# SandAI-org/MagiAttention

Measured on AMD Instinct MI355X. Metric: attention TFLOPS/sec fwd+bwd (whole-job; per-GPU = value/n_gpus); cp scaling at seqlen 64k, higher is better.
Workload: dtype bf16; 1 GPU; dense_causal_64k_h32_d128; seqlen=65536, heads=32, kv_heads=32, head_dim=128, mask=causal, global_batch=1, parallelism=cp1

## Files before the change

### magi_attention/csrc/ffa_bwd.hip

```cpp

#include <hip/hip_runtime.h>
#include <math.h>
#include <stdlib.h>

#include "../../include/magi_ffa.h"
#include "ffa_device.h"

#define BWD_BN 32
#define BWD_BM 32

DEV_INLINE bool wave_alive(int m0, int qe) { return m0 < qe; }

DEV_INLINE void glds16_untracked(const void* gsrc, int lds_byte) {
  const int m0v = __builtin_amdgcn_readfirstlane(lds_byte);
  asm volatile("s_mov_b32 m0, %0\n\ts_nop 0\n\tglobal_load_lds_dwordx4 %1, off"
               :: "s"(m0v), "v"(gsrc) : "memory", "m0");
}

struct BwdParams {
  const bf16_t* dout;
  const bf16_t* q;
  const bf16_t* k;
  const bf16_t* v;
  const void* out;
  const float* lse;
  float* dq;
  float* dk;
  float* dv;
  float* dpsum;
  const int* q_ranges;
  const int* k_ranges;
  const int* attn_type_map;
  int hq, hk, gqa;
  float scale;
  float softcap;
  long long total_q, total_k;
  int head_major;
  int work_nx, work_ny, work_nz;
  int head_mult;
  int head_off;
  int n_heads_launch;
  const int* seg_starts;
};

template <bool OUT_F32>
__global__ __launch_bounds__(256) void bwd_preprocess_kernel(BwdParams p, int d,
                                                             long long n_rows) {
  const long long row = (long long)blockIdx.x * 4 + (threadIdx.x >> 6);
  if (row >= n_rows) return;
  const int lane = threadIdx.x & 63;
  const int per = d / 64;
  const bf16_t* do_p = p.dout + row * d;
  float acc = 0.f;
  for (int e = 0; e < per; ++e) {
    const int idx = lane * per + e;
    const float dov = (float)do_p[idx];
    float ov;
    if (OUT_F32)
      ov = ((const float*)p.out)[row * d + idx];
    else
      ov = (float)((const bf16_t*)p.out)[row * d + idx];
    acc += dov * ov;
  }
#pragma unroll
  for (int s = 32; s > 0; s >>= 1) acc += __shfl_xor(acc, s, 64);
  if (lane == 0) p.dpsum[row] = acc;
}


template <int D, bool HAS_SOFTCAP, int MODE, int WAVES>
__global__ __launch_bounds__(64 * WAVES, WAVES == 8 ? 2 : 1)
void ffa_bwd_dkv_kernel(BwdParams p) {
  static_assert(WAVES == 4 || (WAVES == 8 && D != 192), "unsupported shape");
  constexpr int NBUF = (MODE != 0 && WAVES == 8) ? 3 : 2;
  constexpr bool WANT_DV = MODE != 2;
  constexpr bool WANT_DK = MODE != 1;
  constexpr bool V_IN_LDS = MODE == 0;
  constexpr int DF = D / 16;
  constexpr int DT = D / 32;
  constexpr int ROWB = (D == 192) ? 512 : D * 2;
  constexpr int ROWE = ROWB / 2;
  constexpr int VSLOTS = D / 8;
  constexpr int SW32M = ROWB / 32 - 1;
  auto swz = [](int row, int byte_off) {
    return byte_off ^ ((row & SW32M) << 5);
  };
  const long long work_total =
      (long long)p.work_nx * p.work_ny * p.work_nz;
  const long long grid_span = (long long)gridDim.x * gridDim.y * gridDim.z;
  const long long w_first = blockIdx.x +
      (long long)gridDim.x * (blockIdx.y + (long long)gridDim.y * blockIdx.z);
  for (long long w = w_first; w < work_total; w += grid_span) {
  const int wx = (int)(w % p.work_nx);
  const long long w2 = w / p.work_nx;
  const int wy = (int)(w2 % p.work_ny);
  const int wz = (int)(w2 / p.work_ny);
  const int ri = wz;
  const int hidx = p.head_major ? wx : wy;
  const int h = p.head_off + hidx * p.head_mult;
  const int wb = p.head_major ? wy : wx;
  const int ks = p.k_ranges[2 * ri], ke = p.k_ranges[2 * ri + 1];
  const int nblk0 = ks + wb * (BWD_BN * WAVES);
  if (nblk0 >= ke) continue;
  const int seg0 = p.seg_starts ? p.seg_starts[ri] : ri;
  const int seg1 = p.seg_starts ? p.seg_starts[ri + 1] : ri + 1;
  int qs, qe, atype;

  const int tid = threadIdx.x;
  const int lane = tid & 63;
  const int wave = tid >> 6;
  if (WAVES == 8 && wave >= 4) asm volatile("s_setprio 1");

  const int lo32 = lane & 31;
  const int hi = lane >> 5;

  const int n0 = nblk0 + wave * BWD_BN;
  const bool wave_live = n0 < ke;

  const float sl2 = HAS_SOFTCAP ? p.softcap * 1.4426950408889634f
                                : p.scale * 1.4426950408889634f;
  const float cap_pre = HAS_SOFTCAP ? p.scale / p.softcap : 0.f;
  const float log2e = 1.4426950408889634f;

  const int kh = h / p.gqa;
  const size_t k_pitch = (size_t)p.hk * D;
  const size_t q_pitch = (size_t)p.hq * D;

  constexpr int QITER =
      (V_IN_LDS && D == 128 && WAVES == 8) ? BWD_BM : 2 * BWD_BM;
  constexpr int NSUB = QITER / BWD_BM;
  constexpr int KVLDS = V_IN_LDS ? 2 * WAVES * BWD_BN * ROWB : 0;
  constexpr int LSELDS = V_IN_LDS ? 0 : NBUF * 2 * QITER * 4;
  static_assert(NBUF * 2 * QITER * ROWB + LSELDS + KVLDS <= 163840,
                "LDS budget");
  __shared__ __attribute__((aligned(16))) char smem[
      NBUF * 2 * QITER * ROWB + LSELDS + KVLDS];
  auto lds_q = [&](int buf) -> __bf16* {
    return (__bf16*)(smem + (2 * buf) * QITER * ROWB);
  };
  auto lds_do = [&](int buf) -> __bf16* {
    return (__bf16*)(smem + (2 * buf + 1) * QITER * ROWB);
  };
  auto lds_lse = [&](int buf) -> float* {
    return (float*)(smem + NBUF * 2 * QITER * ROWB + buf * 2 * QITER * 4);
  };
  __bf16* lds_kt = (__bf16*)(smem + NBUF * 2 * QITER * ROWB + LSELDS) +
                   wave * BWD_BN * ROWE;
  __bf16* lds_vt = (__bf16*)(smem + NBUF * 2 * QITER * ROWB + LSELDS +
                             KVLDS / 2) +
                   wave * BWD_BN * ROWE;

  const int krow = n0 + lo32;
  const int kcl = min(krow, ke - 1);
  const bf16_t* kp_row = p.k + (size_t)kcl * k_pitch + (size_t)kh * D + hi * 8;
  bf16x8 kfA[V_IN_LDS ? 1 : DF], vfA[(WANT_DK && !V_IN_LDS) ? DF : 1];
  if constexpr (!V_IN_LDS) {
    const bf16_t* vp = p.v + (size_t)kcl * k_pitch + (size_t)kh * D;
#pragma unroll
    for (int dd = 0; dd < DF; ++dd) {
      kfA[dd] = *(const bf16x8*)(kp_row - hi * 8 + dd * 16 + hi * 8);
      if constexpr (WANT_DK)
        vfA[dd] = *(const bf16x8*)(vp + dd * 16 + hi * 8);
    }
  }
  constexpr int ROWS_PER_GLDS_V = 1024 / ROWB;
  if constexpr (V_IN_LDS) {
#pragma unroll
    for (int gi = 0; gi < BWD_BN / ROWS_PER_GLDS_V; ++gi) {
      const int r0v = ROWS_PER_GLDS_V * gi;
      const int r = r0v + lane / (ROWB / 16);
// ... 268 lines not shown
              else
                bnext = tr16_frag(tbase + rb0 + (dcoln ^ sw0),
                                  tbase + rb1 + (dcoln ^ sw1));
            }
            acc[j >> 1] = __builtin_amdgcn_mfma_f32_32x32x16_bf16(
                (j & 1) ? a1 : a0, bcur, acc[j >> 1], 0, 0, 0);
            bcur = bnext;
          }
        };
        if constexpr (MODE == 1) {
          pipe_mm(do_base, cframe_to_afrag(pv, 0), cframe_to_afrag(pv, 1),
                  acc_dv);
        } else if constexpr (MODE == 2) {
          pipe_mm(q_base, cframe_to_afrag(dsv, 0), cframe_to_afrag(dsv, 1),
                  acc_dk);
        } else {
          bf16x8 pa0 = cframe_to_afrag(pv, 0);
          bf16x8 pa1 = cframe_to_afrag(pv, 1);
          bf16x8 da0 = cframe_to_afrag(dsv, 0);
          bf16x8 da1 = cframe_to_afrag(dsv, 1);
#pragma unroll
          for (int dt = 0; dt < DT; ++dt) {
            const int dcol = (dt * 32 + 16 * qhalf) * 2;
            bf16x8 bdo = tr16_frag(do_base + rb0 + (dcol ^ sw0),
                                   do_base + rb1 + (dcol ^ sw1));
            acc_dv[dt] = __builtin_amdgcn_mfma_f32_32x32x16_bf16(
                pa0, bdo, acc_dv[dt], 0, 0, 0);
            bf16x8 bq = tr16_frag(q_base + rb0 + (dcol ^ sw0),
                                  q_base + rb1 + (dcol ^ sw1));
            acc_dk[dt] = __builtin_amdgcn_mfma_f32_32x32x16_bf16(
                da0, bq, acc_dk[dt], 0, 0, 0);
            bf16x8 bdo1 = tr16_frag(do_base + rb2 + (dcol ^ sw2),
                                    do_base + rb3 + (dcol ^ sw3));
            acc_dv[dt] = __builtin_amdgcn_mfma_f32_32x32x16_bf16(
                pa1, bdo1, acc_dv[dt], 0, 0, 0);
            bf16x8 bq1 = tr16_frag(q_base + rb2 + (dcol ^ sw2),
                                   q_base + rb3 + (dcol ^ sw3));
            acc_dk[dt] = __builtin_amdgcn_mfma_f32_32x32x16_bf16(
                da1, bq1, acc_dk[dt], 0, 0, 0);
          }
        }
      }
    }
    }
    cur = (NBUF == 3) ? (cur == 2 ? 0 : cur + 1) : (cur ^ 1);
  }
  __syncthreads();
  }

  if (wave_live) {
#pragma unroll
  for (int r = 0; r < 16; ++r) {
    const int kr = n0 + crow(r, hi);
    if (kr >= ke) continue;
    float* dkp = p.dk + (size_t)kr * k_pitch + (size_t)kh * D;
    float* dvp = p.dv + (size_t)kr * k_pitch + (size_t)kh * D;
#pragma unroll
    for (int dt = 0; dt < DT; ++dt) {
      if constexpr (WANT_DK) {
        if (acc_dk[dt][r] != 0.f)
          unsafeAtomicAdd(dkp + dt * 32 + lo32, acc_dk[dt][r]);
      }
      if constexpr (WANT_DV) {
        if (acc_dv[dt][r] != 0.f)
          unsafeAtomicAdd(dvp + dt * 32 + lo32, acc_dv[dt][r]);
      }
    }
  }
  }
  if constexpr (MODE == 0) break;
  }
}


template <int D, bool HAS_SOFTCAP, int WAVES>
__global__ __launch_bounds__(64 * WAVES, WAVES == 8 ? 1 : 2)
void ffa_bwd_dq_kernel(BwdParams p) {
  static_assert(WAVES == 4 || (WAVES == 8 && D != 192), "unsupported shape");
  constexpr int NBUF = WAVES == 8 ? 3 : 2;
  constexpr int DF = D / 16;
  constexpr int DT = D / 32;
  constexpr int ROWB = (D == 192) ? 512 : D * 2;
  constexpr int ROWE = ROWB / 2;
  constexpr int VSLOTS = D / 8;
  constexpr int SW32M = ROWB / 32 - 1;
  auto swz = [](int row, int byte_off) {
    return byte_off ^ ((row & SW32M) << 5);
  };
  const long long work_total =
      (long long)p.work_nx * p.work_ny * p.work_nz;
  const long long grid_span = (long long)gridDim.x * gridDim.y * gridDim.z;
  for (long long w = blockIdx.x +
           (long long)gridDim.x * (blockIdx.y + (long long)gridDim.y * blockIdx.z);
       w < work_total; w += grid_span) {
  const int wx = (int)(w % p.work_nx);
  const long long w2 = w / p.work_nx;
  const int wy = (int)(w2 % p.work_ny);
  const int wz = (int)(w2 / p.work_ny);
  const int ri = wz;
  const int h = p.head_major ? wx : wy;
  const int wb_lin = p.head_major ? wy : wx;
  const int qs = p.q_ranges[2 * ri], qe = p.q_ranges[2 * ri + 1];
  const int nqb = (qe - qs + BWD_BM * WAVES - 1) / (BWD_BM * WAVES);
  if (wb_lin >= nqb) continue;
  const int seg0 = p.seg_starts ? p.seg_starts[ri] : ri;
  const int seg1 = p.seg_starts ? p.seg_starts[ri + 1] : ri + 1;
  const int at0 = p.attn_type_map ? p.attn_type_map[seg0] : 0;
  const int wb = (at0 == 1 || at0 == 3) ? nqb - 1 - wb_lin : wb_lin;
  const int mblk0 = qs + wb * (BWD_BM * WAVES);
  int ks, ke, atype;

  const int tid = threadIdx.x;
  const int lane = tid & 63;
  const int wave = tid >> 6;
  if (WAVES == 8 && wave >= 4) asm volatile("s_setprio 1");

  const int lo32 = lane & 31;
  const int hi = lane >> 5;

  const int m0 = mblk0 + wave * BWD_BM;
  const int qrow = m0 + lo32;
  const bool qvalid = qrow < qe && m0 < qe;
  const int qcl = qvalid ? qrow : (qe - 1);

  const float sl2 = HAS_SOFTCAP ? p.softcap * 1.4426950408889634f
                                : p.scale * 1.4426950408889634f;
  const float cap_pre = HAS_SOFTCAP ? p.scale / p.softcap : 0.f;
  const float log2e = 1.4426950408889634f;

  const int kh = h / p.gqa;
  const size_t k_pitch = (size_t)p.hk * D;
  const size_t q_pitch = (size_t)p.hq * D;

  constexpr int KITER = 2 * BWD_BN;
  static_assert(NBUF * 2 * KITER * ROWB <= 163840, "LDS budget");
  __shared__ __attribute__((aligned(16))) char smem[NBUF * 2 * KITER * ROWB];
  auto lds_k = [&](int buf) -> __bf16* {
    return (__bf16*)(smem + (2 * buf) * KITER * ROWB);
  };
  auto lds_v = [&](int buf) -> __bf16* {
    return (__bf16*)(smem + (2 * buf + 1) * KITER * ROWB);
  };

  bf16x8 qf[DF], dof[DF];
  {
    const bf16_t* qp = p.q + (size_t)qcl * q_pitch + (size_t)h * D;
    const bf16_t* dp = p.dout + (size_t)qcl * q_pitch + (size_t)h * D;
#pragma unroll
    for (int dd = 0; dd < DF; ++dd) {
      qf[dd] = *(const bf16x8*)(qp + dd * 16 + hi * 8);
      dof[dd] = *(const bf16x8*)(dp + dd * 16 + hi * 8);
    }
  }
  const float lse_q = qvalid ? p.lse[(size_t)qrow * p.hq + h] : INFINITY;
  const float dpsum_q = qvalid ? p.dpsum[(size_t)qrow * p.hq + h] : 0.f;
  const bool row_live = qvalid && lse_q != INFINITY && lse_q != -INFINITY;

  const int mlast = min(mblk0 + BWD_BM * WAVES, qe) - 1;
  int k_lo = 0, k_hi = 0, wk_lo = 0, wk_hi = 0;
  auto seg_bounds = [&]() {
    k_lo = ks; k_hi = ke;
    if (atype == 1 || atype == 3) k_hi = min(k_hi, mlast + (ke - qe) + 1);
    if (atype == 2 || atype == 3) k_lo = max(k_lo, mblk0 + (ks - qs));
    wk_lo = ks; wk_hi = ke;
    if (atype == 1 || atype == 3)
      wk_hi = min(wk_hi, min(m0 + BWD_BM, qe) - 1 + (ke - qe) + 1);
    if (atype == 2 || atype == 3) wk_lo = max(wk_lo, m0 + (ks - qs));
  };

  f32x16 acc_dq[DT];
#pragma unroll
  for (int dt = 0; dt < DT; ++dt) acc_dq[dt] = (f32x16)(0.f);

  constexpr int ROWS_PER_GLDS = 1024 / ROWB;
  static_assert(KITER / WAVES >= ROWS_PER_GLDS, "stage rows per wave");
  constexpr int GLDS_PER_WAVE = (KITER / WAVES) / ROWS_PER_GLDS;
  auto stage_glds = [&](int buf, int n0x) {
#pragma unroll
    for (int gi = 0; gi < GLDS_PER_WAVE; ++gi) {
      const int r0 = (KITER / WAVES) * wave + ROWS_PER_GLDS * gi;
      const int r = r0 + lane / (ROWB / 16);
      const int c = lane % (ROWB / 16);
      const int kr = min(n0x + r, ke - 1);
      int cs = c ^ ((r & SW32M) << 1);
      if (cs >= VSLOTS) cs = 0;
      const int csw = cs * 8;
      __builtin_amdgcn_global_load_lds(
          (const __attribute__((address_space(1))) unsigned int*)(
              p.k + (size_t)kr * k_pitch + (size_t)kh * D + csw),
          (__attribute__((address_space(3))) unsigned int*)&lds_k(buf)[r0 * ROWE],
          16, 0, 0);
      __builtin_amdgcn_global_load_lds(
          (const __attribute__((address_space(1))) unsigned int*)(
              p.v + (size_t)kr * k_pitch + (size_t)kh * D + csw),
          (__attribute__((address_space(3))) unsigned int*)&lds_v(buf)[r0 * ROWE],
          16, 0, 0);
    }
  };

  constexpr int GOPS = 2 * GLDS_PER_WAVE;
  int cur = 0;
  for (int seg = seg0; seg < seg1; ++seg) {
  ks = p.k_ranges[2 * seg];
  ke = p.k_ranges[2 * seg + 1];
  atype = p.attn_type_map ? p.attn_type_map[seg] : 0;
  if (ke <= ks) continue;
  seg_bounds();
  if (k_lo >= k_hi) continue;
  cur = 0;
  stage_glds(0, k_lo);
  if constexpr (NBUF == 3) stage_glds(1, k_lo + KITER);

  for (int n0 = k_lo; n0 < k_hi; n0 += KITER) {
    pipe_barrier<NBUF == 3 ? GOPS : 0>();
    if constexpr (NBUF == 3) {
      stage_glds(cur == 0 ? 2 : cur - 1, n0 + 2 * KITER);
    } else {
      if (n0 + KITER < k_hi) stage_glds(cur ^ 1, n0 + KITER);
    }
#pragma unroll
    for (int sub = 0; sub < 2; ++sub) {
    const int ns = n0 + sub * BWD_BN;
    if (ns >= k_hi) break;
    const __bf16* lkb = lds_k(cur) + sub * BWD_BN * ROWE;
    const __bf16* lvb = lds_v(cur) + sub * BWD_BN * ROWE;

    if (wave_alive(m0, qe) && ns + BWD_BN > wk_lo && ns < wk_hi) {
      f32x16 sA = (f32x16)(0.f), dpA = (f32x16)(0.f);
#pragma unroll
      for (int dd = 0; dd < DF; ++dd) {
        const int off = swz(lo32, lo32 * ROWB + dd * 32 + hi * 16);
        bf16x8 kf = *(const bf16x8*)((const char*)lkb + off);
        bf16x8 vf = *(const bf16x8*)((const char*)lvb + off);
        sA = __builtin_amdgcn_mfma_f32_32x32x16_bf16(kf, qf[dd], sA, 0, 0, 0);
        dpA = __builtin_amdgcn_mfma_f32_32x32x16_bf16(vf, dof[dd], dpA, 0, 0, 0);
      }

      float dsv[16];
      const bool interior =
          (qrow < qe) && row_live && (ns >= ks) && (ns + BWD_BN <= ke) &&
          !((atype == 1 || atype == 3) && (ns + BWD_BN - 1 > m0 + (ke - qe))) &&
          !((atype == 2 || atype == 3) && (ns < m0 + 31 + (ks - qs)));
      if (__all(interior) && !HAS_SOFTCAP) {
        const float lsc = lse_q * log2e;
#pragma unroll
        for (int r = 0; r < 16; ++r) {
          const float pij = fast_exp2(sA[r] * sl2 - lsc);
          dsv[r] = pij * (dpA[r] - dpsum_q) * p.scale;
        }
      } else {
#pragma unroll
        for (int r = 0; r < 16; ++r) {
          const int kk = ns + crow(r, hi);
          bool ok = row_live && kk < ke && kk >= ks;
          if (atype == 1 || atype == 3) ok = ok && (kk - qrow <= ke - qe);
          if (atype == 2 || atype == 3) ok = ok && (kk - qrow >= ks - qs);
          float sv = sA[r];
          float dscale = p.scale;
          float t;
          if (HAS_SOFTCAP) {
            const float th = tanhf(sv * cap_pre);
            t = th * sl2;
            dscale = p.scale * (1.f - th * th);
          } else {
            t = sv * sl2;
          }
          const float pij = ok ? fast_exp2(t - lse_q * log2e) : 0.f;
          dsv[r] = pij * (dpA[r] - dpsum_q) * dscale;
        }
      }

      bf16x8 dsa0 = cframe_to_afrag(dsv, 0);
      bf16x8 dsa1 = cframe_to_afrag(dsv, 1);
      {
        const int qhalf2 = (lane >> 4) & 1;
        const int jrow = (lane & 15) >> 2;
        const int row0 = 8 * hi + jrow;
        const int row1 = 8 * hi + 4 + jrow;
        const int k_base = (int)(unsigned long long)(
            (__attribute__((address_space(3))) const char*)lkb);
        const int lane8 = (lane & 3) * 8;
        const int sw0 = (row0 & SW32M) << 5;
        const int sw1 = (row1 & SW32M) << 5;
        const int rb0 = row0 * ROWB + lane8;
        const int rb1 = row1 * ROWB + lane8;
        const int sw2 = ((row0 + 16) & SW32M) << 5;
        const int sw3 = ((row1 + 16) & SW32M) << 5;
        const int rb2 = (row0 + 16) * ROWB + lane8;
        const int rb3 = (row1 + 16) * ROWB + lane8;
        bf16x8 bcur = tr16_frag(k_base + rb0 + ((16 * qhalf2 * 2) ^ sw0),
                                k_base + rb1 + ((16 * qhalf2 * 2) ^ sw1));
#pragma unroll
        for (int j = 0; j < 2 * DT; ++j) {
          bf16x8 bnext = bcur;
          if (j + 1 < 2 * DT) {
            const int dcoln = (((j + 1) >> 1) * 32 + 16 * qhalf2) * 2;
            if ((j + 1) & 1)
              bnext = tr16_frag(k_base + rb2 + (dcoln ^ sw2),
                                k_base + rb3 + (dcoln ^ sw3));
            else
              bnext = tr16_frag(k_base + rb0 + (dcoln ^ sw0),
                                k_base + rb1 + (dcoln ^ sw1));
          }
          acc_dq[j >> 1] = __builtin_amdgcn_mfma_f32_32x32x16_bf16(
              (j & 1) ? dsa1 : dsa0, bcur, acc_dq[j >> 1], 0, 0, 0);
          bcur = bnext;
        }
      }
    }
    }
    cur = (NBUF == 3) ? (cur == 2 ? 0 : cur + 1) : (cur ^ 1);
  }
  __syncthreads();
  }

#pragma unroll
  for (int r = 0; r < 16; ++r) {
    const int qr = m0 + crow(r, hi);
    if (qr >= qe) continue;
    float* dst = p.dq + (size_t)qr * q_pitch + (size_t)h * D;
#pragma unroll
    for (int dt = 0; dt < DT; ++dt) {
      const float val = acc_dq[dt][r];
      if (val != 0.f) unsafeAtomicAdd(dst + dt * 32 + lo32, val);
    }
  }
  }
}


extern "C" int magi_ffa_bwd_preprocess(const magi_ffa_bwd_args* a) {
  if (!a || !a->dout || !a->out || !a->dpsum) return -1;
  BwdParams p{};
  p.dout = (const bf16_t*)a->dout;
  p.out = a->out;
  p.dpsum = a->dpsum;
  const long long n_rows = a->total_q * a->hq;
  if (n_rows == 0) return 0;
  dim3 grid((unsigned)((n_rows + 3) / 4)), block(256);
  hipStream_t s = (hipStream_t)a->stream;
  if (a->out_is_fp32)
    hipLaunchKernelGGL((bwd_preprocess_kernel<true>), grid, block, 0, s, p,
                       a->d, n_rows);
  else
    hipLaunchKernelGGL((bwd_preprocess_kernel<false>), grid, block, 0, s, p,
                       a->d, n_rows);
  return (int)hipGetLastError();
}

static int fill_bwd_params(const magi_ffa_bwd_args* a, BwdParams* p) {
  if (!a || !a->dout || !a->q || !a->k || !a->v || !a->lse) return -1;
  if (a->d != 64 && a->d != 128 && a->d != 192) return -2;
  if (a->hq % a->hk != 0) return -3;
  if (a->n_ranges <= 0) return 1;
  p->dout = (const bf16_t*)a->dout;
  p->q = (const bf16_t*)a->q;
  p->k = (const bf16_t*)a->k;
  p->v = (const bf16_t*)a->v;
  p->out = a->out;
  p->lse = a->lse;
  p->dq = a->dq;
  p->dk = a->dk;
  p->dv = a->dv;
  p->dpsum = a->dpsum;
  p->q_ranges = a->q_ranges;
  p->k_ranges = a->k_ranges;
  p->attn_type_map = a->attn_type_map;
  p->hq = a->hq;
  p->hk = a->hk;
  p->gqa = a->hq / a->hk;
  p->scale = a->softmax_scale;
  p->softcap = a->softcap;
  p->total_q = a->total_q;
  p->total_k = a->total_k;
  p->seg_starts = a->seg_starts;
  p->head_mult = 1;
  p->head_off = 0;
  p->n_heads_launch = a->hq;
  if (a->cu_margin & 0xFFFF0000) {
    p->head_mult = (a->cu_margin >> 24) & 0xFF;
    p->head_off = (a->cu_margin >> 16) & 0xFF;
    p->n_heads_launch = a->hq / p->head_mult;
  }
  return 0;
}

static int env_int(const char* name, int dflt) {
  const char* e = getenv(name);
  return e ? atoi(e) : dflt;
}

static dim3 cap_grid(dim3 grid, int margin, int wg_per_cu) {
  if (margin <= 0) return grid;
  const long long total = (long long)grid.x * grid.y * grid.z;
  long long cap = (long long)(256 - margin) * wg_per_cu;
  if (cap < 1) cap = 1;
  if (cap > total) cap = total;
  return dim3((unsigned)cap, 1, 1);
}

struct BwdKnobs {
  int head_major;
  int bigseq;
};

static BwdKnobs dq_knobs(const magi_ffa_bwd_args* a) {
  const int hm = ((long long)a->total_k * a->d * 4 <= (16 << 20)) ? 1 : 0;
  return {env_int("MAGI_BWD_HEAD_MAJOR", hm),
          env_int("MAGI_BWD_DQ_BIGSEQ", 8192)};
}

template <int D>
static void launch_dq(int waves, bool sc, dim3 grid, hipStream_t s,
                      const BwdParams& p) {
#define GO(SC, W)                                                          \
  hipLaunchKernelGGL((ffa_bwd_dq_kernel<D, SC, W>), grid, dim3(64 * W), 0, \
                     s, p)
  if constexpr (D != 192) {
    if (waves == 8) {
      if (sc) GO(true, 8); else GO(false, 8);
      return;
    }
  }
  if (sc) GO(true, 4); else GO(false, 4);
#undef GO
}

extern "C" int magi_ffa_bwd_dq(const magi_ffa_bwd_args* a) {
  BwdParams p;
  int rc = fill_bwd_params(a, &p);
  if (rc) return rc > 0 ? 0 : rc;
  const BwdKnobs knobs = dq_knobs(a);
  p.head_major = knobs.head_major;
  const int W = (a->d != 192 && a->max_seqlen_k >= knobs.bigseq) ? 8 : 4;
  if (a->n_ranges > 65535) return -5;
  const int qspan = BWD_BM * W;
  const int qblocks = (int)((a->total_q + qspan - 1) / qspan);
  dim3 grid = p.head_major ? dim3(a->hq, qblocks, (unsigned)a->n_ranges)
                           : dim3(qblocks, a->hq, (unsigned)a->n_ranges);
  p.work_nx = grid.x; p.work_ny = grid.y; p.work_nz = grid.z;
  grid = cap_grid(grid, a->cu_margin & 0xFFFF, W == 4 ? 2 : 1);
  hipStream_t s = (hipStream_t)a->stream;
  const bool sc = a->softcap > 0.f;
  if (a->d == 64) launch_dq<64>(W, sc, grid, s, p);
  else if (a->d == 192) launch_dq<192>(W, sc, grid, s, p);
  else launch_dq<128>(W, sc, grid, s, p);
  return (int)hipGetLastError();
}

static BwdKnobs dkv_knobs() {
  return {env_int("MAGI_BWD_HEAD_MAJOR", 1), env_int("MAGI_BWD_BIGSEQ", 1024)};
}

template <int D, int MODE>
static void launch_dkv(int waves, bool sc, dim3 grid, hipStream_t s,
                       const BwdParams& p) {
#define GO(SC, W)                                                        \
  hipLaunchKernelGGL((ffa_bwd_dkv_kernel<D, SC, MODE, W>), grid,         \
                     dim3(64 * W), 0, s, p)
  if constexpr (D != 192) {
    if (waves == 8) {
      if (sc) GO(true, 8); else GO(false, 8);
      return;
    }
  }
// ... 49 lines not shown
```

### magi_attention/csrc/ffa_device.h

```cpp
#pragma once

#include <hip/hip_runtime.h>

using f32x16 = __attribute__((ext_vector_type(16))) float;
using bf16x8 = __attribute__((ext_vector_type(8))) __bf16;
using bf16_t = __bf16;

#define DEV_INLINE __device__ __forceinline__

template <int VM>
DEV_INLINE void pipe_barrier() {
  asm volatile("s_waitcnt vmcnt(%0)\n\ts_waitcnt lgkmcnt(0)\n\ts_barrier"
               :: "n"(VM) : "memory");
}

DEV_INLINE float warp_xor32(float v) { return __shfl_xor(v, 32, 64); }

DEV_INLINE unsigned pack_bf16_pair(float lo, float hi) {
  unsigned r;
  asm("v_cvt_pk_bf16_f32 %0, %1, %2" : "=v"(r) : "v"(lo), "v"(hi));
  return r;
}

DEV_INLINE float fast_exp2(float x) { return __builtin_amdgcn_exp2f(x); }

DEV_INLINE int crow(int r, int hi) { return (r & 3) + 8 * (r >> 2) + 4 * hi; }

DEV_INLINE bf16x8 tr16_frag(int a0, int a1) {
  typedef __attribute__((ext_vector_type(4))) __bf16 bf16x4_;
  bf16x4_ v0 = __builtin_amdgcn_ds_read_tr16_b64_v4bf16(
      (__attribute__((address_space(3))) bf16x4_*)(unsigned)a0);
  bf16x4_ v1 = __builtin_amdgcn_ds_read_tr16_b64_v4bf16(
      (__attribute__((address_space(3))) bf16x4_*)(unsigned)a1);
  union {
    bf16x4_ h[2];
    bf16x8 v;
  } r;
  r.h[0] = v0;
  r.h[1] = v1;
  return r.v;
}

DEV_INLINE bf16x8 cframe_to_afrag(const float* val, int tt) {
  unsigned c0 = pack_bf16_pair(val[8 * tt + 0], val[8 * tt + 1]);
  unsigned c1 = pack_bf16_pair(val[8 * tt + 2], val[8 * tt + 3]);
  unsigned c2 = pack_bf16_pair(val[8 * tt + 4], val[8 * tt + 5]);
  unsigned c3 = pack_bf16_pair(val[8 * tt + 6], val[8 * tt + 7]);
  {
    auto r2 = __builtin_amdgcn_permlane32_swap(c0, c2, false, false);
    c0 = r2[0];
    c2 = r2[1];
  }
  {
    auto r2 = __builtin_amdgcn_permlane32_swap(c1, c3, false, false);
    c1 = r2[0];
    c3 = r2[1];
  }
  union {
    unsigned u[4];
    bf16x8 v;
  } cvt;
  cvt.u[0] = c0;
  cvt.u[1] = c1;
  cvt.u[2] = c2;
  cvt.u[3] = c3;
  return cvt.v;
}


DEV_INLINE unsigned char to_fp8(float x) {
  union {
    short s;
    unsigned char b[2];
  } r;
  r.s = __builtin_amdgcn_cvt_pk_fp8_f32(x, 0.f, 0, false);
  return r.b[0];
}

DEV_INLINE long cframe_to_afrag_fp8(const float* val, int tt) {
  union {
    unsigned char b[4];
    unsigned u;
  } A, B;
#pragma unroll
  for (int j = 0; j < 4; ++j) {
    A.b[j] = to_fp8(val[8 * tt + j]);
    B.b[j] = to_fp8(val[8 * tt + 4 + j]);
  }
  auto r2 = __builtin_amdgcn_permlane32_swap(A.u, B.u, false, false);
  return ((long)(unsigned)r2[1] << 32) | (unsigned)r2[0];
}
```

### magi_attention/csrc/ffa_fwd.hip

```cpp

#include <hip/hip_runtime.h>
#include <math.h>

#include "../../include/magi_ffa.h"
#include "ffa_device.h"

#define FFA_BM 128
#define FFA_BN 32
#define LOCK_GRAN 128

struct FwdParams {
  const bf16_t* q;
  const bf16_t* k;
  const bf16_t* v;
  float* out_f32;
  bf16_t* out_bf16;
  float* lse;
  const int* q_ranges;
  const int* k_ranges;
  const int* attn_type_map;
  int* locks;
  float* max_logits;
  const int* qk_starts;
  int hq, hk, gqa;
  int head_major;
  int work_nx, work_ny, work_nz;
  int n_lock_slots;
  float scale;
  float softcap;
  long long total_q, total_k;
};

template <int D, bool HAS_SOFTCAP, bool ATOMIC, bool OUT_BF16, int WAVES,
          int NBUF = 2>
__global__ __launch_bounds__(64 * WAVES, 8 / WAVES) void ffa_fwd_kernel(FwdParams p) {
  constexpr int DF = D / 16;
  constexpr int DT = D / 32;
  const long long work_total =
      (long long)p.work_nx * p.work_ny * p.work_nz;
  const long long grid_span = (long long)gridDim.x * gridDim.y * gridDim.z;
  for (long long w = blockIdx.x +
           (long long)gridDim.x * (blockIdx.y + (long long)gridDim.y * blockIdx.z);
       w < work_total; w += grid_span) {
  const int wx = (int)(w % p.work_nx);
  const long long w2 = w / p.work_nx;
  const int wy = (int)(w2 % p.work_ny);
  const int wz = (int)(w2 / p.work_ny);
  const int ri = p.head_major ? wz : wy;
  const int h = p.head_major ? wx : wz;
  const int mb = p.head_major ? wy : wx;
  const int qs = p.q_ranges[2 * ri], qe = p.q_ranges[2 * ri + 1];
  const int m0 = qs + mb * (32 * WAVES);
  if (m0 >= qe) continue;
  const int seg0 = p.qk_starts ? p.qk_starts[ri] : ri;
  const int seg1 = p.qk_starts ? p.qk_starts[ri + 1] : ri + 1;
  int ks, ke, atype;

  const int lane = threadIdx.x & 63;
  const int wave = threadIdx.x >> 6;
  if (WAVES == 8 && wave >= 4) asm volatile("s_setprio 1");

  const int lo32 = lane & 31;
  const int hi = lane >> 5;

  const int q0 = m0 + wave * 32;
  const int qrow = q0 + lo32;
  const bool qvalid = (qrow < qe) && (q0 < qe);
  const bool qvalid_any = q0 < qe;
  const int qclamp = qvalid ? qrow : (qe - 1);

  const float sl2 = HAS_SOFTCAP ? p.softcap * 1.4426950408889634f
                                : p.scale * 1.4426950408889634f;
  const float cap_pre = HAS_SOFTCAP ? p.scale / p.softcap : 0.f;

  int n_lo = 0, n_hi = 0, b_lo = 0, b_hi = 0;
  auto seg_bounds = [&]() {
    n_lo = ks; n_hi = ke;
    if (ke > ks && q0 < qe) {
      const int qhiw = min(q0 + 31, qe - 1);
      if (atype == 1 || atype == 3) n_hi = min(n_hi, qhiw + (ke - qe) + 1);
      if (atype == 2 || atype == 3) n_lo = max(n_lo, q0 + (ks - qs));
    } else {
      n_hi = n_lo;
    }
    b_lo = ks; b_hi = ke;
    if (ke > ks && m0 < qe) {
      const int qhib = min(m0 + 32 * WAVES - 1, qe - 1);
      if (atype == 1 || atype == 3) b_hi = min(b_hi, qhib + (ke - qe) + 1);
      if (atype == 2 || atype == 3) b_lo = max(b_lo, m0 + (ks - qs));
    } else {
      b_hi = b_lo;
    }
  };
  constexpr int ROWB = (D == 192) ? 512 : D * 2;
  constexpr int ROWE = ROWB / 2;
  constexpr int VSLOTS = D / 8;
  constexpr int SW32M = ROWB / 32 - 1;
  auto swz = [](int row, int byte_off) {
    return byte_off ^ ((row & SW32M) << 5);
  };
  constexpr int KITER = 2 * FFA_BN;
  __shared__ __attribute__((aligned(16))) char fsmem[NBUF * 2 * KITER * ROWB];
  auto lds_k = [&](int buf) -> __bf16* {
    return (__bf16*)(fsmem + (2 * buf) * KITER * ROWB);
  };
  auto lds_v = [&](int buf) -> __bf16* {
    return (__bf16*)(fsmem + (2 * buf + 1) * KITER * ROWB);
  };

  bf16x8 qf[DF];
  {
    const bf16_t* qp = p.q + (size_t)qclamp * p.hq * D + (size_t)h * D;
#pragma unroll
    for (int dd = 0; dd < DF; ++dd)
      qf[dd] = *(const bf16x8*)(qp + dd * 16 + hi * 8);
  }

  const int kh = h / p.gqa;
  const size_t k_pitch = (size_t)p.hk * D;
  const bf16_t* kbase = p.k + (size_t)kh * D;
  const bf16_t* vbase = p.v + (size_t)kh * D;

  float m_run = -INFINITY;
  float l_run = 0.f;
  f32x16 acc_o[DT];
#pragma unroll
  for (int dt = 0; dt < DT; ++dt) acc_o[dt] = (f32x16)(0.f);

  constexpr int ROWS_PER_GLDS = 1024 / ROWB;
  static_assert(KITER / WAVES >= ROWS_PER_GLDS, "stage rows per wave");
  constexpr int GLDS_PER_WAVE = (KITER / WAVES) / ROWS_PER_GLDS;
  constexpr int GOPS = 2 * GLDS_PER_WAVE;
  auto stage_glds = [&](int buf, int n0x) {
#pragma unroll
    for (int gi = 0; gi < GLDS_PER_WAVE; ++gi) {
      const int r0 = (KITER / WAVES) * wave + ROWS_PER_GLDS * gi;
      const int r = r0 + lane / (ROWB / 16);
      const int c = lane % (ROWB / 16);
      const int kr = min(n0x + r, ke - 1);
      int cs = c ^ ((r & SW32M) << 1);
      if (cs >= VSLOTS) cs = 0;
      const int csw = cs * 8;
      __builtin_amdgcn_global_load_lds(
          (const __attribute__((address_space(1))) unsigned int*)(
              kbase + (size_t)kr * k_pitch + csw),
          (__attribute__((address_space(3))) unsigned int*)&lds_k(buf)[r0 * ROWE],
          16, 0, 0);
      __builtin_amdgcn_global_load_lds(
          (const __attribute__((address_space(1))) unsigned int*)(
              vbase + (size_t)kr * k_pitch + csw),
          (__attribute__((address_space(3))) unsigned int*)&lds_v(buf)[r0 * ROWE],
          16, 0, 0);
    }
  };

  int cur = 0;

  auto sub_body = [&](int ns, const __bf16* lkb, const __bf16* lvb) {
    const bool live = (ns + FFA_BN > n_lo) && (ns < n_hi) && qvalid_any;
    if (!live) return;

    f32x16 s = (f32x16)(0.f);
    {
#pragma unroll
      for (int dd = 0; dd < DF; ++dd) {
        bf16x8 kf = *(const bf16x8*)(
            (const char*)lkb + swz(lo32, lo32 * ROWB + dd * 32 + hi * 16));
        s = __builtin_amdgcn_mfma_f32_32x32x16_bf16(kf, qf[dd], s, 0, 0, 0);
      }
    }

    const bool interior =
        (q0 + 31 < qe) && (ns >= n_lo) && (ns + FFA_BN <= n_hi) &&
        !((atype == 1 || atype == 3) && (ns + FFA_BN - 1 > q0 + (ke - qe))) &&
        !((atype == 2 || atype == 3) && (ns < q0 + 31 + (ks - qs)));
    float t[16];
    float mx = -INFINITY;
    if (interior) {
#pragma unroll
      for (int r = 0; r < 16; ++r) {
        float sv = s[r];
        if (HAS_SOFTCAP) sv = tanhf(sv * cap_pre);
        t[r] = sv * sl2;
        mx = fmaxf(mx, t[r]);
      }
    } else {
#pragma unroll
      for (int r = 0; r < 16; ++r) {
        const int kk = ns + crow(r, hi);
        bool ok = qvalid && (kk >= n_lo) && (kk < n_hi);
        if (atype == 1 || atype == 3) ok = ok && (kk - qrow <= ke - qe);
        if (atype == 2 || atype == 3) ok = ok && (kk - qrow >= ks - qs);
        float sv = s[r];
        if (HAS_SOFTCAP) sv = tanhf(sv * cap_pre);
        t[r] = ok ? sv * sl2 : -INFINITY;
        mx = fmaxf(mx, t[r]);
      }
    }
    mx = fmaxf(mx, warp_xor32(mx));

    const float m_new = fmaxf(m_run, mx);
    const float defer_thr = p.max_logits ? 0.f : 8.f;
    const bool need_rescale =
        (m_new > m_run + defer_thr) ||
        (m_run == -INFINITY && m_new != -INFINITY);
    float m_use;
    float alpha;
    if (!__any(need_rescale)) {
      m_use = (m_run == -INFINITY) ? 0.f : m_run;
      alpha = 1.f;
    } else {
      m_use = (m_new == -INFINITY) ? 0.f : m_new;
      alpha = (m_run == -INFINITY) ? 0.f : fast_exp2(m_run - m_use);
      m_run = m_new;
    }

    float pr[16];
    float psum = 0.f;
#pragma unroll
    for (int r = 0; r < 16; ++r) {
      pr[r] = fast_exp2(t[r] - m_use);
      psum += pr[r];
    }
    l_run = l_run * alpha + (psum + warp_xor32(psum));

    if (__any(alpha != 1.f)) {
#pragma unroll
      for (int r = 0; r < 16; ++r) {
        const int src = crow(r, hi);
        const float aq = __uint_as_float(
            __builtin_amdgcn_ds_bpermute(src << 2, __float_as_uint(alpha)));
#pragma unroll
        for (int dt = 0; dt < DT; ++dt) acc_o[dt][r] *= aq;
      }
    }

    bf16x8 pa[2];
#pragma unroll
    for (int tt = 0; tt < 2; ++tt) {
      unsigned c0 = pack_bf16_pair(pr[8 * tt + 0], pr[8 * tt + 1]);
      unsigned c1 = pack_bf16_pair(pr[8 * tt + 2], pr[8 * tt + 3]);
      unsigned c2 = pack_bf16_pair(pr[8 * tt + 4], pr[8 * tt + 5]);
      unsigned c3 = pack_bf16_pair(pr[8 * tt + 6], pr[8 * tt + 7]);
      {
        auto r2 = __builtin_amdgcn_permlane32_swap(c0, c2, false, false);
        c0 = r2[0];
        c2 = r2[1];
      }
      {
        auto r2 = __builtin_amdgcn_permlane32_swap(c1, c3, false, false);
        c1 = r2[0];
        c3 = r2[1];
      }
      union {
        unsigned u[4];
        bf16x8 v;
      } cvt;
      cvt.u[0] = c0;
      cvt.u[1] = c1;
      cvt.u[2] = c2;
      cvt.u[3] = c3;
      pa[tt] = cvt.v;
    }

    {
      const int qhalf = (lane >> 4) & 1;
      const int jrow = (lane & 15) >> 2;
      const int v_base = (int)(unsigned long long)(
          (__attribute__((address_space(3))) const char*)lvb);
      const int lane8 = (lane & 3) * 8;
#pragma unroll
      for (int tt = 0; tt < 2; ++tt) {
        const int row0 = 16 * tt + 8 * hi + jrow;
        const int row1 = row0 + 4;
        const int sw0 = (row0 & SW32M) << 5;
        const int sw1 = (row1 & SW32M) << 5;
        const int rb0 = v_base + row0 * ROWB + lane8;
        const int rb1 = v_base + row1 * ROWB + lane8;
#pragma unroll
        for (int dt = 0; dt < DT; ++dt) {
          const int dcol = (dt * 32 + 16 * qhalf) * 2;
          bf16x8 bv = tr16_frag(rb0 + (dcol ^ sw0), rb1 + (dcol ^ sw1));
          acc_o[dt] =
              __builtin_amdgcn_mfma_f32_32x32x16_bf16(pa[tt], bv, acc_o[dt], 0, 0, 0);
        }
      }
    }
  };

  bool any_seg = false;
  for (int seg = seg0; seg < seg1; ++seg) {
    ks = p.k_ranges[2 * seg];
    ke = p.k_ranges[2 * seg + 1];
    atype = p.attn_type_map ? p.attn_type_map[seg] : 0;
    if (ke <= ks) continue;
    seg_bounds();
    if (b_lo >= b_hi) continue;
    any_seg = true;
    cur = 0;
    stage_glds(0, b_lo);
    if constexpr (NBUF == 3) stage_glds(1, b_lo + KITER);
    for (int n0 = b_lo; n0 < b_hi; n0 += KITER) {
      pipe_barrier<NBUF == 3 ? GOPS : 0>();
      if constexpr (NBUF == 3) {
        stage_glds(cur == 0 ? 2 : cur - 1, n0 + 2 * KITER);
      } else {
        if (n0 + KITER < b_hi) stage_glds(cur ^ 1, n0 + KITER);
      }
#pragma unroll
      for (int sub = 0; sub < 2; ++sub) {
        const int ns = n0 + sub * FFA_BN;
        if (ns >= b_hi) break;
        sub_body(ns, lds_k(cur) + sub * FFA_BN * ROWE,
                 lds_v(cur) + sub * FFA_BN * ROWE);
      }
      cur = (NBUF == 3) ? (cur == 2 ? 0 : cur + 1) : (cur ^ 1);
    }
    __syncthreads();
  }
  if (any_seg) {

  if (p.max_logits) {
    float ml = m_run * 0.6931471805599453f;
#pragma unroll
    for (int off = 32; off; off >>= 1)
      ml = fmaxf(ml, __shfl_xor(ml, off, 64));
    if (lane == 0 && ml != -INFINITY)
      unsafeAtomicMax(p.max_logits + h, ml);
  }
  const float lse_new =
      (l_run > 0.f) ? (m_run + __log2f(l_run)) * 0.6931471805599453f : -INFINITY;
  const float inv_l = (l_run > 0.f) ? 1.f / l_run : 0.f;

  const size_t out_row_pitch = (size_t)p.hq * D;

  if (!ATOMIC) {
    if (l_run > 0.f && qvalid && hi == 0)
      p.lse[(size_t)qrow * p.hq + h] = lse_new;
#pragma unroll
    for (int r = 0; r < 16; ++r) {
      const int src = crow(r, hi);
      const float ilq = __uint_as_float(
          __builtin_amdgcn_ds_bpermute(src << 2, __float_as_uint(inv_l)));
      const int qr = q0 + src;
      const bool valid = (qr < qe) && ilq > 0.f;
      if (!valid) continue;
      const size_t base = (size_t)qr * out_row_pitch + (size_t)h * D;
#pragma unroll
      for (int dt = 0; dt < DT; ++dt) {
        const float val = acc_o[dt][r] * ilq;
        if (OUT_BF16)
          p.out_bf16[base + dt * 32 + lo32] = (bf16_t)val;
        else
          p.out_f32[base + dt * 32 + lo32] = val;
      }
    }
  } else {

  const int row_last = min(m0 + 32 * WAVES, qe) - 1;
  const int s0 = m0 / LOCK_GRAN, s1 = row_last / LOCK_GRAN;
  if (threadIdx.x == 0) {
    for (int sl = s0; sl <= s1; ++sl) {
      int* lk = p.locks + (size_t)sl * p.hq + h;
      int expected = 0;
      while (!__hip_atomic_compare_exchange_strong(
          lk, &expected, 1, __ATOMIC_ACQUIRE, __ATOMIC_RELAXED,
          __HIP_MEMORY_SCOPE_AGENT))
        expected = 0;
    }
  }
  __syncthreads();

  float lse_prev = -INFINITY;
  if (qvalid) lse_prev = p.lse[(size_t)qrow * p.hq + h];
  float lse_m;
  {
    const float a = fmaxf(lse_prev, lse_new);
    const float b = fminf(lse_prev, lse_new);
    lse_m = (a == -INFINITY) ? -INFINITY : a + log1pf(expf(b - a));
  }
  const float w_prev = (lse_prev == -INFINITY) ? 0.f : expf(lse_prev - lse_m);
  const float w_new = (lse_new == -INFINITY) ? 0.f : expf(lse_new - lse_m) * inv_l;

  if (qvalid && lse_m != -INFINITY && hi == 0)
    p.lse[(size_t)qrow * p.hq + h] = lse_m;

#pragma unroll
  for (int r = 0; r < 16; ++r) {
    const int src = crow(r, hi);
    const float wp = __uint_as_float(
        __builtin_amdgcn_ds_bpermute(src << 2, __float_as_uint(w_prev)));
    const float wn = __uint_as_float(
        __builtin_amdgcn_ds_bpermute(src << 2, __float_as_uint(w_new)));
    const int qr = q0 + src;
    if (qr >= qe || (wp == 0.f && wn == 0.f)) continue;
    const size_t base = (size_t)qr * out_row_pitch + (size_t)h * D;
#pragma unroll
    for (int dt = 0; dt < DT; ++dt) {
      float* ptr = p.out_f32 + base + dt * 32 + lo32;
      const float prev = (wp > 0.f) ? wp * (*ptr) : 0.f;
      *ptr = prev + wn * acc_o[dt][r];
    }
  }

  asm volatile("s_waitcnt vmcnt(0)" ::: "memory");
  __syncthreads();
  if (threadIdx.x == 0) {
    asm volatile("s_waitcnt vmcnt(0)" ::: "memory");
    for (int sl = s1; sl >= s0; --sl)
      __hip_atomic_store(p.locks + (size_t)sl * p.hq + h, 0, __ATOMIC_RELEASE,
                         __HIP_MEMORY_SCOPE_AGENT);
  }
  }
  }
  }
}

__global__ void probe_mfma_kernel(const bf16_t* a, const bf16_t* b, float* d) {
  const int lane = threadIdx.x & 63;
  const int lo32 = lane & 31, hi = lane >> 5;
  bf16x8 af = *(const bf16x8*)(a + lo32 * 16 + hi * 8);
  bf16x8 bf;
  union {
    unsigned short u[8];
    bf16x8 v;
  } bu;
  for (int e = 0; e < 8; ++e)
    bu.u[e] = *(const unsigned short*)(b + (hi * 8 + e) * 32 + lo32);
  bf = bu.v;
  f32x16 acc = (f32x16)(0.f);
  acc = __builtin_amdgcn_mfma_f32_32x32x16_bf16(af, bf, acc, 0, 0, 0);
  for (int r = 0; r < 16; ++r) d[(size_t)crow(r, hi) * 32 + lo32] = acc[r];
}

__global__ void probe_lane_kernel(const unsigned* in, unsigned* out) {
  const int lane = threadIdx.x & 63;
  unsigned a = in[lane];
  unsigned b = in[lane] + 1000u;
  auto r2 = __builtin_amdgcn_permlane32_swap(a, b, false, false);
  out[lane] = r2[0];
  out[64 + lane] = r2[1];
  out[128 + lane] =
      __builtin_amdgcn_ds_bpermute((lane & 31) << 2, in[lane]);
}

extern "C" int magi_probe_lane(const void* in, void* out, void* stream) {
  hipLaunchKernelGGL(probe_lane_kernel, dim3(1), dim3(64), 0,
                     (hipStream_t)stream, (const unsigned*)in, (unsigned*)out);
  return (int)hipGetLastError();
}

extern "C" int magi_probe_mfma(const void* a, const void* b, void* d,
                               void* stream) {
  hipLaunchKernelGGL(probe_mfma_kernel, dim3(1), dim3(64), 0,
                     (hipStream_t)stream, (const bf16_t*)a, (const bf16_t*)b,
                     (float*)d);
  return (int)hipGetLastError();
}

template <int D, int W, int NB>
static int launch_fwd_d(const magi_ffa_fwd_args* a, const FwdParams& p,
                        dim3 grid, dim3 block, hipStream_t stream) {
  const bool sc = a->softcap > 0.f;
  const bool atomic = !a->disable_atomic_reduction;
  const bool obf16 = !a->out_is_fp32;
  if (atomic && obf16) return -10;
#define LAUNCH(SC, AT, OB)                                                 \
  hipLaunchKernelGGL((ffa_fwd_kernel<D, SC, AT, OB, W, NB>), grid, block,  \
                     0, stream, p)
  if (atomic) {
// ... 119 lines not shown
```

Baseline: 613.5 TFLOPS/s.

## Use untracked LDS loads, software-pipeline MFMA fragments, reverse causal block order

Both kernels now stage K/V through an inline-asm global_load_lds that the compiler does not track, so its conservative waits go away; vmcnt is drained explicitly before each segment barrier. The LDS fragment reads feeding the MFMAs are double-buffered and interleaved with sched_group_barrier hints, and Q/dO/LSE values are pinned in VGPRs. The forward kernel also reverses the query-block order for causal masks so the heaviest blocks launch first, which should improve load balance. The risks are races from the untracked loads if the manual waits are wrong, and higher register pressure.

```diff
diff --git a/magi_attention/csrc/ffa_bwd.hip b/magi_attention/csrc/ffa_bwd.hip
--- a/magi_attention/csrc/ffa_bwd.hip
+++ b/magi_attention/csrc/ffa_bwd.hip
@@ -10,12 +10,6 @@
 #define BWD_BM 32
 
 DEV_INLINE bool wave_alive(int m0, int qe) { return m0 < qe; }
-
-DEV_INLINE void glds16_untracked(const void* gsrc, int lds_byte) {
-  const int m0v = __builtin_amdgcn_readfirstlane(lds_byte);
-  asm volatile("s_mov_b32 m0, %0\n\ts_nop 0\n\tglobal_load_lds_dwordx4 %1, off"
-               :: "s"(m0v), "v"(gsrc) : "memory", "m0");
-}
 
 struct BwdParams {
   const bf16_t* dout;
@@ -590,8 +584,8 @@
       dof[dd] = *(const bf16x8*)(dp + dd * 16 + hi * 8);
     }
   }
-  const float lse_q = qvalid ? p.lse[(size_t)qrow * p.hq + h] : INFINITY;
-  const float dpsum_q = qvalid ? p.dpsum[(size_t)qrow * p.hq + h] : 0.f;
+  float lse_q = qvalid ? p.lse[(size_t)qrow * p.hq + h] : INFINITY;
+  float dpsum_q = qvalid ? p.dpsum[(size_t)qrow * p.hq + h] : 0.f;
   const bool row_live = qvalid && lse_q != INFINITY && lse_q != -INFINITY;
 
   const int mlast = min(mblk0 + BWD_BM * WAVES, qe) - 1;
@@ -613,6 +607,8 @@
   constexpr int ROWS_PER_GLDS = 1024 / ROWB;
   static_assert(KITER / WAVES >= ROWS_PER_GLDS, "stage rows per wave");
   constexpr int GLDS_PER_WAVE = (KITER / WAVES) / ROWS_PER_GLDS;
+  const int smem_byte = (int)(unsigned long long)(
+      (__attribute__((address_space(3))) const char*)smem);
   auto stage_glds = [&](int buf, int n0x) {
 #pragma unroll
     for (int gi = 0; gi < GLDS_PER_WAVE; ++gi) {
@@ -623,16 +619,10 @@
       int cs = c ^ ((r & SW32M) << 1);
       if (cs >= VSLOTS) cs = 0;
       const int csw = cs * 8;
-      __builtin_amdgcn_global_load_lds(
-          (const __attribute__((address_space(1))) unsigned int*)(
-              p.k + (size_t)kr * k_pitch + (size_t)kh * D + csw),
-          (__attribute__((address_space(3))) unsigned int*)&lds_k(buf)[r0 * ROWE],
-          16, 0, 0);
-      __builtin_amdgcn_global_load_lds(
-          (const __attribute__((address_space(1))) unsigned int*)(
-              p.v + (size_t)kr * k_pitch + (size_t)kh * D + csw),
-          (__attribute__((address_space(3))) unsigned int*)&lds_v(buf)[r0 * ROWE],
-          16, 0, 0);
+      const int lk = smem_byte + (2 * buf * KITER + r0) * ROWB;
+      glds16_untracked(p.k + (size_t)kr * k_pitch + (size_t)kh * D + csw, lk);
+      glds16_untracked(p.v + (size_t)kr * k_pitch + (size_t)kh * D + csw,
+                       lk + KITER * ROWB);
     }
   };
 
@@ -648,6 +638,13 @@
   cur = 0;
   stage_glds(0, k_lo);
   if constexpr (NBUF == 3) stage_glds(1, k_lo + KITER);
+#pragma unroll
+  for (int dd = 0; dd < DF; ++dd) {
+    pin_vgpr(qf[dd]);
+    pin_vgpr(dof[dd]);
+  }
+  pin_vgpr(lse_q);
+  pin_vgpr(dpsum_q);
 
   for (int n0 = k_lo; n0 < k_hi; n0 += KITER) {
     pipe_barrier<NBUF == 3 ? GOPS : 0>();
@@ -665,13 +662,27 @@
 
     if (wave_alive(m0, qe) && ns + BWD_BN > wk_lo && ns < wk_hi) {
       f32x16 sA = (f32x16)(0.f), dpA = (f32x16)(0.f);
-#pragma unroll
-      for (int dd = 0; dd < DF; ++dd) {
-        const int off = swz(lo32, lo32 * ROWB + dd * 32 + hi * 16);
-        bf16x8 kf = *(const bf16x8*)((const char*)lkb + off);
-        bf16x8 vf = *(const bf16x8*)((const char*)lvb + off);
-        sA = __builtin_amdgcn_mfma_f32_32x32x16_bf16(kf, qf[dd], sA, 0, 0, 0);
-        dpA = __builtin_amdgcn_mfma_f32_32x32x16_bf16(vf, dof[dd], dpA, 0, 0, 0);
+      {
+        const int off0 = swz(lo32, lo32 * ROWB + hi * 16);
+        bf16x8 kf = *(const bf16x8*)((const char*)lkb + off0);
+        bf16x8 vf = *(const bf16x8*)((const char*)lvb + off0);
+        __builtin_amdgcn_sched_group_barrier(0x100, 2, 0);
+#pragma unroll
+        for (int dd = 0; dd < DF; ++dd) {
+          bf16x8 kn = kf, vn = vf;
+          if (dd + 1 < DF) {
+            const int off = swz(lo32, lo32 * ROWB + (dd + 1) * 32 + hi * 16);
+            kn = *(const bf16x8*)((const char*)lkb + off);
+            vn = *(const bf16x8*)((const char*)lvb + off);
+            __builtin_amdgcn_sched_group_barrier(0x100, 2, 0);
+          }
+          sA = __builtin_amdgcn_mfma_f32_32x32x16_bf16(kf, qf[dd], sA, 0, 0, 0);
+          dpA =
+              __builtin_amdgcn_mfma_f32_32x32x16_bf16(vf, dof[dd], dpA, 0, 0, 0);
+          __builtin_amdgcn_sched_group_barrier(0x008, 2, 0);
+          kf = kn;
+          vf = vn;
+        }
       }
 
       float dsv[16];
@@ -728,6 +739,7 @@
         const int rb3 = (row1 + 16) * ROWB + lane8;
         bf16x8 bcur = tr16_frag(k_base + rb0 + ((16 * qhalf2 * 2) ^ sw0),
                                 k_base + rb1 + ((16 * qhalf2 * 2) ^ sw1));
+        __builtin_amdgcn_sched_group_barrier(0x100, 2, 0);
 #pragma unroll
         for (int j = 0; j < 2 * DT; ++j) {
           bf16x8 bnext = bcur;
@@ -739,9 +751,11 @@
             else
               bnext = tr16_frag(k_base + rb0 + (dcoln ^ sw0),
                                 k_base + rb1 + (dcoln ^ sw1));
+            __builtin_amdgcn_sched_group_barrier(0x100, 2, 0);
           }
           acc_dq[j >> 1] = __builtin_amdgcn_mfma_f32_32x32x16_bf16(
               (j & 1) ? dsa1 : dsa0, bcur, acc_dq[j >> 1], 0, 0, 0);
+          __builtin_amdgcn_sched_group_barrier(0x008, 1, 0);
           bcur = bnext;
         }
       }
@@ -749,6 +763,7 @@
     }
     cur = (NBUF == 3) ? (cur == 2 ? 0 : cur + 1) : (cur ^ 1);
   }
+  drain_vm();
   __syncthreads();
   }
 
diff --git a/magi_attention/csrc/ffa_device.h b/magi_attention/csrc/ffa_device.h
--- a/magi_attention/csrc/ffa_device.h
+++ b/magi_attention/csrc/ffa_device.h
@@ -12,6 +12,21 @@
 DEV_INLINE void pipe_barrier() {
   asm volatile("s_waitcnt vmcnt(%0)\n\ts_waitcnt lgkmcnt(0)\n\ts_barrier"
                :: "n"(VM) : "memory");
+}
+
+DEV_INLINE void glds16_untracked(const void* gsrc, int lds_byte) {
+  const int m0v = __builtin_amdgcn_readfirstlane(lds_byte);
+  asm volatile("s_mov_b32 m0, %0\n\ts_nop 0\n\tglobal_load_lds_dwordx4 %1, off"
+               :: "s"(m0v), "v"(gsrc) : "memory", "m0");
+}
+
+DEV_INLINE void drain_vm() {
+  asm volatile("s_waitcnt vmcnt(0)" ::: "memory");
+}
+
+template <class T>
+DEV_INLINE void pin_vgpr(T& x) {
+  asm volatile("" : "+v"(x));
 }
 
 DEV_INLINE float warp_xor32(float v) { return __shfl_xor(v, 32, 64); }
diff --git a/magi_attention/csrc/ffa_fwd.hip b/magi_attention/csrc/ffa_fwd.hip
--- a/magi_attention/csrc/ffa_fwd.hip
+++ b/magi_attention/csrc/ffa_fwd.hip
@@ -48,12 +48,16 @@
   const int wz = (int)(w2 / p.work_ny);
   const int ri = p.head_major ? wz : wy;
   const int h = p.head_major ? wx : wz;
-  const int mb = p.head_major ? wy : wx;
+  const int mb_lin = p.head_major ? wy : wx;
   const int qs = p.q_ranges[2 * ri], qe = p.q_ranges[2 * ri + 1];
-  const int m0 = qs + mb * (32 * WAVES);
-  if (m0 >= qe) continue;
+  const int nqb = (qe - qs + 32 * WAVES - 1) / (32 * WAVES);
+  if (mb_lin >= nqb) continue;
   const int seg0 = p.qk_starts ? p.qk_starts[ri] : ri;
   const int seg1 = p.qk_starts ? p.qk_starts[ri + 1] : ri + 1;
+  const int at0 =
+      (p.attn_type_map && seg0 < seg1) ? p.attn_type_map[seg0] : 0;
+  const int mb = (at0 == 1 || at0 == 3) ? nqb - 1 - mb_lin : mb_lin;
+  const int m0 = qs + mb * (32 * WAVES);
   int ks, ke, atype;
 
   const int lane = threadIdx.x & 63;
@@ -131,6 +135,8 @@
   static_assert(KITER / WAVES >= ROWS_PER_GLDS, "stage rows per wave");
   constexpr int GLDS_PER_WAVE = (KITER / WAVES) / ROWS_PER_GLDS;
   constexpr int GOPS = 2 * GLDS_PER_WAVE;
+  const int fsmem_byte = (int)(unsigned long long)(
+      (__attribute__((address_space(3))) const char*)fsmem);
   auto stage_glds = [&](int buf, int n0x) {
 #pragma unroll
     for (int gi = 0; gi < GLDS_PER_WAVE; ++gi) {
@@ -141,16 +147,9 @@
       int cs = c ^ ((r & SW32M) << 1);
       if (cs >= VSLOTS) cs = 0;
       const int csw = cs * 8;
-      __builtin_amdgcn_global_load_lds(
-          (const __attribute__((address_space(1))) unsigned int*)(
-              kbase + (size_t)kr * k_pitch + csw),
-          (__attribute__((address_space(3))) unsigned int*)&lds_k(buf)[r0 * ROWE],
-          16, 0, 0);
-      __builtin_amdgcn_global_load_lds(
-          (const __attribute__((address_space(1))) unsigned int*)(
-              vbase + (size_t)kr * k_pitch + csw),
-          (__attribute__((address_space(3))) unsigned int*)&lds_v(buf)[r0 * ROWE],
-          16, 0, 0);
+      const int lk = fsmem_byte + (2 * buf * KITER + r0) * ROWB;
+      glds16_untracked(kbase + (size_t)kr * k_pitch + csw, lk);
+      glds16_untracked(vbase + (size_t)kr * k_pitch + csw, lk + KITER * ROWB);
     }
   };
 
@@ -269,21 +268,30 @@
       const int v_base = (int)(unsigned long long)(
           (__attribute__((address_space(3))) const char*)lvb);
       const int lane8 = (lane & 3) * 8;
-#pragma unroll
-      for (int tt = 0; tt < 2; ++tt) {
+      auto vfrag = [&](int j) {
+        const int tt = j / DT, dt = j % DT;
         const int row0 = 16 * tt + 8 * hi + jrow;
         const int row1 = row0 + 4;
         const int sw0 = (row0 & SW32M) << 5;
         const int sw1 = (row1 & SW32M) << 5;
         const int rb0 = v_base + row0 * ROWB + lane8;
         const int rb1 = v_base + row1 * ROWB + lane8;
-#pragma unroll
-        for (int dt = 0; dt < DT; ++dt) {
-          const int dcol = (dt * 32 + 16 * qhalf) * 2;
-          bf16x8 bv = tr16_frag(rb0 + (dcol ^ sw0), rb1 + (dcol ^ sw1));
-          acc_o[dt] =
-              __builtin_amdgcn_mfma_f32_32x32x16_bf16(pa[tt], bv, acc_o[dt], 0, 0, 0);
+        const int dcol = (dt * 32 + 16 * qhalf) * 2;
+        return tr16_frag(rb0 + (dcol ^ sw0), rb1 + (dcol ^ sw1));
+      };
+      bf16x8 bcur = vfrag(0);
+      __builtin_amdgcn_sched_group_barrier(0x100, 2, 0);
+#pragma unroll
+      for (int j = 0; j < 2 * DT; ++j) {
+        bf16x8 bnext = bcur;
+        if (j + 1 < 2 * DT) {
+          bnext = vfrag(j + 1);
+          __builtin_amdgcn_sched_group_barrier(0x100, 2, 0);
         }
+        acc_o[j % DT] = __builtin_amdgcn_mfma_f32_32x32x16_bf16(
+            pa[j / DT], bcur, acc_o[j % DT], 0, 0, 0);
+        __builtin_amdgcn_sched_group_barrier(0x008, 1, 0);
+        bcur = bnext;
       }
     }
   };
@@ -300,6 +308,8 @@
     cur = 0;
     stage_glds(0, b_lo);
     if constexpr (NBUF == 3) stage_glds(1, b_lo + KITER);
+#pragma unroll
+    for (int dd = 0; dd < DF; ++dd) pin_vgpr(qf[dd]);
     for (int n0 = b_lo; n0 < b_hi; n0 += KITER) {
       pipe_barrier<NBUF == 3 ? GOPS : 0>();
       if constexpr (NBUF == 3) {
@@ -316,6 +326,7 @@
       }
       cur = (NBUF == 3) ? (cur == 2 ? 0 : cur + 1) : (cur ^ 1);
     }
+    drain_vm();
     __syncthreads();
   }
   if (any_seg) {
```

Result: faster. 642.5 TFLOPS/s, median of 6 (+4.7%).
